# yifangao112/DinoUNet

Hardware: AMD Instinct MI355X
Metric: 2D slices/sec training, dinounet_l 512x512 bf16 (higher is better)
Workload: dtype bf16; 1 GPU; dinounet_l train step (fwd+loss+bwd+clip+SGD), 512x512x3 slices, batch 8/GPU, frozen ViT + adapter + FAPM + U-Net decoder, random-init weights; global_batch=8, parallelism=dp1

## Files before the change

### dinounet_amd/csrc/elementwise.hip

```cpp
#include <stdlib.h>
#include "common.h"
#include "dwconv_plan.h"

namespace {

__host__ int grid_1d(long total) {
  long g = (total + 255) / 256;
  if (g < 1) g = 1;
  if (g > 65535L * 8) g = 65535L * 8;
  return (int)g;
}

#define GRID_STRIDE(i, total) for (long i = (long)blockIdx.x * 256 + threadIdx.x; i < (total); i += (long)gridDim.x * 256)

struct PyrPix { int b, s0, Hs, Ws, yo, xo; };
__device__ __forceinline__ PyrPix pyr_decode(long p, int H, int W) {
  const int n = (H * W) >> 2, N = 21 * n;
  PyrPix q;
  q.b = (int)(p / N);
  int t = (int)(p - (long)q.b * N);
  if (t < 16 * n) { q.s0 = 0; q.Hs = 2 * H; q.Ws = 2 * W; }
  else if (t < 20 * n) { q.s0 = 16 * n; q.Hs = H; q.Ws = W; t -= 16 * n; }
  else { q.s0 = 20 * n; q.Hs = H >> 1; q.Ws = W >> 1; t -= 20 * n; }
  q.yo = t / q.Ws; q.xo = t - q.yo * q.Ws;
// ... 266 lines not shown
  }
}

__global__ __launch_bounds__(256) void dwconv_wgrad_finalize_kernel(const float* __restrict__ part, float* __restrict__ dw,
                                                                    float* __restrict__ db, int blocks, int C, int accum) {
  __shared__ float red[8][33];
  const int col = threadIdx.x & 31, sl = threadIdx.x >> 5;
  const int i = blockIdx.x * 32 + col;
  float acc = 0.f;
  if (i < C * 10)
    for (int b = sl; b < blocks; b += 8) acc += part[(long)b * C * 10 + i];
  red[sl][col] = acc;
  __syncthreads();
  if (sl == 0 && i < C * 10) {
    float t = 0.f;
#pragma unroll
    for (int q = 0; q < 8; q++) t += red[q][col];
    const int k = i / C, c = i - k * C;
    if (k < 9) dw[c * 9 + k] = accum ? dw[c * 9 + k] + t : t;
    else if (db) db[c] = accum ? db[c] + t : t;
  }
}

template <typename T>
__global__ __launch_bounds__(256) void maxpool_fwd_kernel(const T* __restrict__ x, T* __restrict__ y, uint8_t* __restrict__ idx,
                                                          int B, int H, int W, int C, int Ho, int Wo, long total) {
  constexpr int V = Elem<T>::VEC;
  const int cvn = C / V;
  GRID_STRIDE(i, total) {
    const int c0 = (int)(i % cvn) * V;
    long t = i / cvn;
    const int xo = (int)(t % Wo); t /= Wo;
    const int yo = (int)(t % Ho);
    const int b = (int)(t / Ho);
    float best[V]; int bi[V];
#pragma unroll
    for (int j = 0; j < V; j++) { best[j] = -INFINITY; bi[j] = 0; }
#pragma unroll
    for (int dy = 0; dy < 3; dy++) {
      const int yi = yo * 2 - 1 + dy;
      if (yi < 0 || yi >= H) continue;
#pragma unroll
      for (int dx = 0; dx < 3; dx++) {
        const int xi = xo * 2 - 1 + dx;
        if (xi < 0 || xi >= W) continue;
        Vec16<T> v = as_vec<T>(*(const uint4*)(x + (((long)b * H + yi) * W + xi) * C + c0));
// ... 1 lines not shown
        for (int j = 0; j < V; j++) {
          float f = to_f32(v.v[j]);
          if (f > best[j]) { best[j] = f; bi[j] = dy * 3 + dx; }
        }
      }
    }
    const long off = (((long)b * Ho + yo) * Wo + xo) * C + c0;
    Vec16<T> o;
#pragma unroll
    for (int j = 0; j < V; j++) o.v[j] = from_f32<T>(best[j]);
    *(uint4*)(y + off) = as_u4(o);
    if (idx) {
#pragma unroll
      for (int j = 0; j < V; j++) idx[off + j] = (uint8_t)bi[j];
    }
  }
}

template <typename T>
__global__ __launch_bounds__(256) void maxpool_bwd_kernel(const uint8_t* __restrict__ idx, const T* __restrict__ dy,
                                                          T* __restrict__ dx, int B, int H, int W, int C, int Ho, int Wo,
                                                          long total) {
  constexpr int V = Elem<T>::VEC;
  const int cvn = C / V;
  GRID_STRIDE(i, total) {
    const int c0 = (int)(i % cvn) * V;
    long t = i / cvn;
    const int xi = (int)(t % W); t /= W;
    const int yi = (int)(t % H);
    const int b = (int)(t / H);
    float acc[V];
#pragma unroll
    for (int j = 0; j < V; j++) acc[j] = 0.f;
#pragma unroll
    for (int dy_ = 0; dy_ < 3; dy_++) {
      const int ty = yi + 1 - dy_;
      if (ty < 0 || (ty & 1)) continue;
      const int yo = ty >> 1;
      if (yo >= Ho) continue;
#pragma unroll
      for (int dx_ = 0; dx_ < 3; dx_++) {
        const int tx = xi + 1 - dx_;
        if (tx < 0 || (tx & 1)) continue;
        const int xo = tx >> 1;
        if (xo >= Wo) continue;
        const long off = (((long)b * Ho + yo) * Wo + xo) * C + c0;
        Vec16<T> g = as_vec<T>(*(const uint4*)(dy + off));
#pragma unroll
        for (int j = 0; j < V; j++)
          if (idx[off + j] == dy_ * 3 + dx_) acc[j] += to_f32(g.v[j]);
      }
    }
    Vec16<T> o;
#pragma unroll
    for (int j = 0; j < V; j++) o.v[j] = from_f32<T>(acc[j]);
    *(uint4*)(dx + (((long)b * H + yi) * W + xi) * C + c0) = as_u4(o);
  }
}

template <typename TS, typename T, int V>
__global__ __launch_bounds__(256) void bilinear_add_kernel(const TS* __restrict__ src, long lds_, const T* __restrict__ base,
                                                           long ldb, T* __restrict__ out, long ldo, int B, int Hs, int Ws, int Ho,
                                                           int Wo, int C, long total) {
  const int cvn = C / V;
  const float sh = (float)Hs / (float)Ho, sw = (float)Ws / (float)Wo;
  auto load = [&](const TS* p, float* v) {
    if constexpr (sizeof(TS) == 2 && V == 8) {
      const bf16x8 t = __builtin_bit_cast(bf16x8, *(const uint4*)p);
#pragma unroll
      for (int j = 0; j < 8; j++) v[j] = (float)t[j];
    } else if constexpr (sizeof(TS) == 4 && V % 4 == 0) {
#pragma unroll
      for (int j = 0; j < V; j += 4) { const float4 t = *(const float4*)(p + j); v[j] = t.x; v[j + 1] = t.y; v[j + 2] = t.z; v[j + 3] = t.w; }
    } else {
// ... 294 lines not shown
__global__ __launch_bounds__(256) void se_scale_kernel(const T* __restrict__ x, long ldx, const float* __restrict__ gate,
                                                       const T* __restrict__ sc, long ldsc, T* __restrict__ y, long ldy, long P, int C,
                                                       long total) {
  constexpr int V = Elem<T>::VEC;
  const int cvn = C / V;
  GRID_STRIDE(i, total) {
    const int c0 = (int)(i % cvn) * V;
    const long pix = i / cvn;
    const int b = (int)(pix / P);
    Vec16<T> t = as_vec<T>(*(const uint4*)(x + pix * ldx + c0));
    Vec16<T> o;
    if (sc) {
      Vec16<T> s2 = as_vec<T>(*(const uint4*)(sc + pix * ldsc + c0));
#pragma unroll
      for (int j = 0; j < V; j++) o.v[j] = from_f32<T>(to_f32(t.v[j]) * gate[(long)b * C + c0 + j] + to_f32(s2.v[j]));
    } else {
#pragma unroll
      for (int j = 0; j < V; j++) o.v[j] = from_f32<T>(to_f32(t.v[j]) * gate[(long)b * C + c0 + j]);
    }
    *(uint4*)(y + pix * ldy + c0) = as_u4(o);
  }
}

__global__ __launch_bounds__(1024) void se_gate_bwd_kernel(const float* __restrict__ dsum, const float* __restrict__ sums, float invP,
                                                           const float* __restrict__ gate, const float* __restrict__ hidden,
                                                           const float* __restrict__ W1, const float* __restrict__ W2,
                                                           float* __restrict__ dpool, float* __restrict__ dW1, float* __restrict__ db1,
                                                           float* __restrict__ dW2, float* __restrict__ db2, int B, int C, int R, int Bc) {
  extern __shared__ float sm[];
  float* dgp = sm;
  float* pooled = dgp + Bc * C;
  float* h = pooled + Bc * C;
  float* dhp = h + Bc * R;
  const int tid = threadIdx.x;
  for (int b0 = 0; b0 < B; b0 += Bc) {
    const int nb = min(Bc, B - b0);
    for (int i = tid; i < nb * C; i += 1024) {
      const long gi = (long)b0 * C + i;
      const float g = gate[gi];
      dgp[i] = dsum[gi * 2] * g * (1.f - g);
      pooled[i] = sums[gi * 2] * invP;
    }
    for (int i = tid; i < nb * R; i += 1024) h[i] = hidden[(long)b0 * R + i];
    __syncthreads();
    for (int i = tid; i < nb * R; i += 1024) {
      const int bl = i / R, r = i - bl * R;
      float acc = 0.f;
      for (int c = 0; c < C; c++) acc += W2[c * R + r] * dgp[bl * C + c];
      dhp[i] = h[i] > 0.f ? acc : 0.f;
    }
    __syncthreads();
    for (int i = tid; i < C * R; i += 1024) {
      float a2 = 0.f, a1 = 0.f;
      { const int c = i / R, r = i - c * R; for (int bl = 0; bl < nb; bl++) a2 += dgp[bl * C + c] * h[bl * R + r]; }
      { const int r = i / C, c = i - r * C; for (int bl = 0; bl < nb; bl++) a1 += dhp[bl * R + r] * pooled[bl * C + c]; }
      dW2[i] = b0 ? dW2[i] + a2 : a2;
      dW1[i] = b0 ? dW1[i] + a1 : a1;
    }
    for (int c = tid; c < C; c += 1024) {
      float a = 0.f;
      for (int bl = 0; bl < nb; bl++) a += dgp[bl * C + c];
      db2[c] = b0 ? db2[c] + a : a;
    }
    for (int r = tid; r < R; r += 1024) {
      float a = 0.f;
      for (int bl = 0; bl < nb; bl++) a += dhp[bl * R + r];
      db1[r] = b0 ? db1[r] + a : a;
    }
    for (int i = tid; i < nb * C; i += 1024) {
      const int bl = i / C, c = i - bl * C;
      float acc = 0.f;
      for (int r = 0; r < R; r++) acc += W1[r * C + c] * dhp[bl * R + r];
      dpool[(long)b0 * C + i] = acc * invP;
    }
    __syncthreads();
  }
}

template <typename T>
__global__ __launch_bounds__(256) void se_scale_bwd_kernel(const T* __restrict__ dy, long lddy, const float* __restrict__ gate,
                                                           const float* __restrict__ dpool, T* __restrict__ dx, long lddx, long P,
                                                           int C, long total) {
  constexpr int V = Elem<T>::VEC;
  const int cvn = C / V;
  GRID_STRIDE(i, total) {
    const int c0 = (int)(i % cvn) * V;
    const long pix = i / cvn;
    const int b = (int)(pix / P);
    Vec16<T> t = as_vec<T>(*(const uint4*)(dy + pix * lddy + c0));
    Vec16<T> o;
#pragma unroll
    for (int j = 0; j < V; j++) o.v[j] = from_f32<T>(to_f32(t.v[j]) * gate[(long)b * C + c0 + j] + dpool[(long)b * C + c0 + j]);
    *(uint4*)(dx + pix * lddx + c0) = as_u4(o);
  }
}
// ... 56 lines not shown

void du_dwconv_row_wgrad(const DwconvPlan& plan, int dtype, const void* x, const void* dz, float* dw, float* db, int64_t ld, int64_t bs,
                         int B, int H, int W, int C, float* part, hipStream_t st) {
  if (dtype == DU_BF16) dwconv_row_wgrad_launch<bf16_t>(plan, (const bf16_t*)x, (const bf16_t*)dz, dw, db, ld, bs, B, H, W, C, part, st);
  else dwconv_row_wgrad_launch<float>(plan, (const float*)x, (const float*)dz, dw, db, ld, bs, B, H, W, C, part, st);
  hipLaunchKernelGGL(dwconv_wgrad_finalize_kernel, dim3((C * 10 + 31) / 32), dim3(256), 0, st, (const float*)part, dw, db, plan.rows, C, 0);
}

extern "C" int du_maxpool3x3s2_fwd(int dtype, const void* x, void* y, uint8_t* idx, int B, int H, int W, int C, void* stream) {
  hipStream_t st = (hipStream_t)stream;
  const int v = dtype == DU_BF16 ? 8 : 4;
  if (!x || !y || B <= 0 || C % v) return DU_ERR_BAD_ARG;
  const int Ho = (H + 2 - 3) / 2 + 1, Wo = (W + 2 - 3) / 2 + 1;
  long total = (long)B * Ho * Wo * (C / v);
  DISPATCH_T(dtype,
             hipLaunchKernelGGL(maxpool_fwd_kernel<bf16_t>, dim3(grid_1d(total)), dim3(256), 0, st, (const bf16_t*)x, (bf16_t*)y, idx, B, H, W, C, Ho, Wo, total),
             hipLaunchKernelGGL(maxpool_fwd_kernel<float>, dim3(grid_1d(total)), dim3(256), 0, st, (const float*)x, (float*)y, idx, B, H, W, C, Ho, Wo, total));
  return du_check_launch();
}

extern "C" int du_maxpool3x3s2_bwd(int dtype, const uint8_t* idx, const void* dy, void* dx, int B, int H, int W, int C, void* stream) {
  hipStream_t st = (hipStream_t)stream;
  const int v = dtype == DU_BF16 ? 8 : 4;
  if (!idx || !dy || !dx || B <= 0 || C % v) return DU_ERR_BAD_ARG;
  const int Ho = (H + 2 - 3) / 2 + 1, Wo = (W + 2 - 3) / 2 + 1;
  long total = (long)B * H * W * (C / v);
  DISPATCH_T(dtype,
             hipLaunchKernelGGL(maxpool_bwd_kernel<bf16_t>, dim3(grid_1d(total)), dim3(256), 0, st, idx, (const bf16_t*)dy, (bf16_t*)dx, B, H, W, C, Ho, Wo, total),
             hipLaunchKernelGGL(maxpool_bwd_kernel<float>, dim3(grid_1d(total)), dim3(256), 0, st, idx, (const float*)dy, (float*)dx, B, H, W, C, Ho, Wo, total));
  return du_check_launch();
}

extern "C" int du_bilinear_add_fwd(int src_dtype, int dtype, const void* src, int64_t lds_, const void* base, int64_t ldb, void* out,
                                   int64_t ldo, int B, int Hs, int Ws, int Ho, int Wo, int C, void* stream) {
  hipStream_t st = (hipStream_t)stream;
  if (!src || !out || B <= 0 || C % 4) return DU_ERR_BAD_ARG;
  const bool v8 = dtype == DU_BF16 && C % 8 == 0 && lds_ % 8 == 0 && ldo % 8 == 0 && (!base || ldb % 8 == 0) &&
                  ((((uintptr_t)src) | ((uintptr_t)out) | ((uintptr_t)base)) & 15) == 0;
  const int V = v8 ? 8 : 4;
  long total = (long)B * Ho * Wo * (C / V);
  dim3 g(grid_1d(total)), b(256);
#define BL_LAUNCH(TS, T, VV) hipLaunchKernelGGL((bilinear_add_kernel<TS, T, VV>), g, b, 0, st, (const TS*)src, lds_, (const T*)base, ldb, (T*)out, ldo, B, Hs, Ws, Ho, Wo, C, total)
  if (src_dtype == DU_F32 && dtype == DU_F32) BL_LAUNCH(float, float, 4);
  else if (src_dtype == DU_F32 && dtype == DU_BF16) { if (v8) BL_LAUNCH(float, bf16_t, 8); else BL_LAUNCH(float, bf16_t, 4); }
  else if (src_dtype == DU_BF16 && dtype == DU_BF16) { if (v8) BL_LAUNCH(bf16_t, bf16_t, 8); else BL_LAUNCH(bf16_t, bf16_t, 4); }
  else return DU_ERR_BAD_ARG;
#undef BL_LAUNCH
// ... 170 lines not shown
}

extern "C" int du_se_scale_fwd(int dtype, const void* x, int64_t ldx, const float* gate, const void* shortcut, int64_t ldsc, void* y,
                               int64_t ldy, int B, int64_t P, int C, void* stream) {
  hipStream_t st = (hipStream_t)stream;
  const int v = dtype == DU_BF16 ? 8 : 4;
  if (!x || !gate || !y || B <= 0 || P <= 0 || C % v || ldx % v || ldy % v || (shortcut && ldsc % v)) return DU_ERR_BAD_ARG;
  long total = (long)B * P * (C / v);
  DISPATCH_T(dtype,
             hipLaunchKernelGGL(se_scale_kernel<bf16_t>, dim3(grid_1d(total)), dim3(256), 0, st, (const bf16_t*)x, ldx, gate, (const bf16_t*)shortcut, ldsc, (bf16_t*)y, ldy, (long)P, C, total),
             hipLaunchKernelGGL(se_scale_kernel<float>, dim3(grid_1d(total)), dim3(256), 0, st, (const float*)x, ldx, gate, (const float*)shortcut, ldsc, (float*)y, ldy, (long)P, C, total));
  return du_check_launch();
}

extern "C" int du_se_gate_bwd(const float* dsum, const float* sums, float inv_count, const float* gate, const float* hidden,
                              const float* W1, const float* W2, float* dpool, float* dW1, float* db1, float* dW2, float* db2, int B, int C,
                              int R, void* stream) {
  hipStream_t st = (hipStream_t)stream;
  if (!dsum || !sums || !gate || !hidden || !W1 || !W2 || !dpool || !dW1 || !db1 || !dW2 || !db2 || B <= 0 || C <= 0 || R <= 0)
    return DU_ERR_BAD_ARG;
  int Bc = (int)(8000 / (long)(C + R));
  if (Bc < 1) return DU_ERR_UNSUPPORTED;
  if (Bc > B) Bc = B;
  hipLaunchKernelGGL(se_gate_bwd_kernel, dim3(1), dim3(1024), (size_t)2 * Bc * (C + R) * sizeof(float), st, dsum, sums, inv_count, gate, hidden,
                     W1, W2, dpool, dW1, db1, dW2, db2, B, C, R, Bc);
  return du_check_launch();
}

extern "C" int du_se_scale_bwd(int dtype, const void* dy, int64_t lddy, const float* gate, const float* dpool, void* dx, int64_t lddx,
                               int B, int64_t P, int C, void* stream) {
  hipStream_t st = (hipStream_t)stream;
  const int v = dtype == DU_BF16 ? 8 : 4;
  if (!dy || !gate || !dpool || !dx || B <= 0 || P <= 0 || C % v || lddy % v || lddx % v) return DU_ERR_BAD_ARG;
  long total = (long)B * P * (C / v);
  DISPATCH_T(dtype,
             hipLaunchKernelGGL(se_scale_bwd_kernel<bf16_t>, dim3(grid_1d(total)), dim3(256), 0, st, (const bf16_t*)dy, lddy, gate, dpool, (bf16_t*)dx, lddx, (long)P, C, total),
             hipLaunchKernelGGL(se_scale_bwd_kernel<float>, dim3(grid_1d(total)), dim3(256), 0, st, (const float*)dy, lddy, gate, dpool, (float*)dx, lddx, (long)P, C, total));
  return du_check_launch();
}

namespace {
__global__ __launch_bounds__(256) void window_accumulate_kernel(const float* __restrict__ logits, const float* __restrict__ gauss,
                                                                const int* __restrict__ coords, float* __restrict__ pred,
                                                                float* __restrict__ npred, int nb, int K, int ph, int pw, int D, int H,
                                                                int W) {
  const long per = (long)ph * pw, total = (long)nb * per;
  GRID_STRIDE(i, total) {
    const int b = (int)(i / per);
// ... 315 lines not shown
```

### dinounet_amd/csrc/norm.hip

```cpp
#include "common.h"
#include "ln_bwd_row.h"

int g_ln_rows2 = 1;

namespace {

template <typename TI, typename TO, int MAXV>
__global__ __launch_bounds__(256) void layernorm_fwd_kernel(const TI* __restrict__ x, long ldx, const float* __restrict__ w,
                                                            const float* __restrict__ b, TO* __restrict__ y, long ldy,
                                                            float* __restrict__ mean_out, float* __restrict__ rstd_out,
                                                            long rows, int D, float eps) {
  constexpr int VI = Elem<TI>::VEC;
  const int lane = threadIdx.x & 63;
  const long row = (long)blockIdx.x * 4 + (threadIdx.x >> 6);
  if (row >= rows) return;
  const int nvec = D / VI;
  float v[MAXV][VI];
  float s = 0.f;
#pragma unroll
  for (int i = 0; i < MAXV; i++) {
    int vi = lane + i * 64;
    if (vi < nvec) {
      Vec16<TI> t = as_vec<TI>(*(const uint4*)(x + row * ldx + (long)vi * VI));
#pragma unroll
      for (int j = 0; j < VI; j++) { v[i][j] = to_f32(t.v[j]); s += v[i][j]; }
    } else {
#pragma unroll
      for (int j = 0; j < VI; j++) v[i][j] = 0.f;
    }
  }
  const float mean = wave_sum(s) / (float)D;
  float s2 = 0.f;
#pragma unroll
  for (int i = 0; i < MAXV; i++) {
    int vi = lane + i * 64;
    if (vi < nvec) {
#pragma unroll
      for (int j = 0; j < VI; j++) { float d = v[i][j] - mean; s2 += d * d; }
    }
  }
  const float rstd = rsqrtf(wave_sum(s2) / (float)D + eps);
  if (lane == 0) {
    if (mean_out) mean_out[row] = mean;
    if (rstd_out) rstd_out[row] = rstd;
  }
#pragma unroll
  for (int i = 0; i < MAXV; i++) {
    int vi = lane + i * 64;
    if (vi < nvec) {
      const int c0 = vi * VI;
#pragma unroll
      for (int j = 0; j < VI; j++) y[row * ldy + c0 + j] = from_f32<TO>((v[i][j] - mean) * rstd * w[c0 + j] + b[c0 + j]);
    }
  }
}

template <typename TI, typename TO, int MAXV>
__global__ __launch_bounds__(256) void layernorm_fwd2_kernel(const TI* __restrict__ x, long ldx, const float* __restrict__ w,
                                                             const float* __restrict__ b, TO* __restrict__ y, long ldy,
                                                             float* __restrict__ mean_out, float* __restrict__ rstd_out,
                                                             long rows, int D, float eps) {
  constexpr int VI = Elem<TI>::VEC;
  const int lane = threadIdx.x & 63;
  const long row0 = ((long)blockIdx.x * 4 + (threadIdx.x >> 6)) * 2;
  if (row0 >= rows) return;
  const bool two = row0 + 1 < rows;
  const int nvec = D / VI;
  float v[2][MAXV][VI];
  float s[2] = {0.f, 0.f};
#pragma unroll
  for (int u = 0; u < 2; u++)
#pragma unroll
    for (int i = 0; i < MAXV; i++) {
      const int vi = lane + i * 64;
      if (vi < nvec && (u == 0 || two)) {
        Vec16<TI> t = as_vec<TI>(*(const uint4*)(x + (row0 + u) * ldx + (long)vi * VI));
#pragma unroll
        for (int j = 0; j < VI; j++) { v[u][i][j] = to_f32(t.v[j]); s[u] += v[u][i][j]; }
      } else {
#pragma unroll
        for (int j = 0; j < VI; j++) v[u][i][j] = 0.f;
      }
    }
  float mean[2], rstd[2];
#pragma unroll
  for (int u = 0; u < 2; u++) mean[u] = wave_sum(s[u]) / (float)D;
#pragma unroll
  for (int u = 0; u < 2; u++) {
    float s2 = 0.f;
#pragma unroll
    for (int i = 0; i < MAXV; i++) {
      const int vi = lane + i * 64;
      if (vi < nvec) {
#pragma unroll
        for (int j = 0; j < VI; j++) { const float d = v[u][i][j] - mean[u]; s2 += d * d; }
      }
    }
    rstd[u] = rsqrtf(wave_sum(s2) / (float)D + eps);
  }
  if (lane == 0) {
    if (mean_out) { mean_out[row0] = mean[0]; if (two) mean_out[row0 + 1] = mean[1]; }
    if (rstd_out) { rstd_out[row0] = rstd[0]; if (two) rstd_out[row0 + 1] = rstd[1]; }
  }
#pragma unroll
  for (int i = 0; i < MAXV; i++) {
    const int vi = lane + i * 64;
    if (vi < nvec) {
      const int c0 = vi * VI;
#pragma unroll
      for (int u = 0; u < 2; u++) {
        if (u == 1 && !two) break;
#pragma unroll
        for (int j = 0; j < VI; j++) y[(row0 + u) * ldy + c0 + j] = from_f32<TO>((v[u][i][j] - mean[u]) * rstd[u] * w[c0 + j] + b[c0 + j]);
      }
    }
  }
}

template <typename T, int MAXV>
__global__ __launch_bounds__(256) void layernorm_bwd_dx_kernel(const T* __restrict__ x, const T* __restrict__ dy,
                                                               const float* __restrict__ w, const float* __restrict__ mean,
                                                               const float* __restrict__ rstd, T* __restrict__ dx, long rows, int D,
                                                               const T* __restrict__ dres) {
  constexpr int VI = Elem<T>::VEC;
  const int lane = threadIdx.x & 63;
  const long row = (long)blockIdx.x * 4 + (threadIdx.x >> 6);
  if (row >= rows) return;
  const int nvec = D / VI;
  const float mu = mean[row], rs = rstd[row];
  float xh[MAXV][VI], g[MAXV][VI];
  float c1 = 0.f, c2 = 0.f;
#pragma unroll
  for (int i = 0; i < MAXV; i++) {
    int vi = lane + i * 64;
    if (vi < nvec) {
      Vec16<T> tx = as_vec<T>(*(const uint4*)(x + row * (long)D + (long)vi * VI));
// ... 565 lines not shown
  if (i >= n) return;
  const float m = sums[i * 2] * inv_count;
  float var = sums[i * 2 + 1] * inv_count - m * m;
  var = var > 0.f ? var : 0.f;
  mean[i] = m;
  rstd[i] = rsqrtf(var + eps);
  if (run_mean) {
    run_mean[i] = (1.f - momentum) * run_mean[i] + momentum * m;
    run_var[i] = (1.f - momentum) * run_var[i] + momentum * var * unbias;
  }
}

__global__ __launch_bounds__(256) void norm_param_grads_kernel(const float* __restrict__ bs, float* __restrict__ dw, float* __restrict__ db,
                                                               int G, int C) {
  const int c = blockIdx.x * 256 + threadIdx.x;
  if (c >= C) return;
  float a = 0.f, b = 0.f;
  for (int g = 0; g < G; g++) { b += bs[((long)g * C + c) * 2]; a += bs[((long)g * C + c) * 2 + 1]; }
  dw[c] = a; db[c] = b;
}

int grid_for(long total) { long g = (total + 255) / 256; return (int)(g > 8192 ? 8192 : (g < 1 ? 1 : g)); }

template <typename TI, typename TO>
int ln_fwd_dispatch(const void* x, long ldx, const float* w, const float* b, void* y, long ldy, float* m, float* r, long rows,
                    int D, float eps, hipStream_t st) {
  const int nvec = D / Elem<TI>::VEC;
  const int maxv = (nvec + 63) / 64;
  dim3 grid((unsigned)((rows + 3) / 4)), block(256);
  static int wave_slots = 0;
  if (!wave_slots) {
    int dev = 0; hipDeviceProp_t prop;
    wave_slots = (hipGetDevice(&dev) == hipSuccess && hipGetDeviceProperties(&prop, dev) == hipSuccess) ? 32 * prop.multiProcessorCount : 8192;
  }
  if (g_ln_rows2 && maxv <= 4 && (g_ln_rows2 > 1 || (rows > wave_slots && rows <= 2L * wave_slots))) {
    dim3 grid2((unsigned)((rows + 7) / 8));
#define LN2_LAUNCH(MV) hipLaunchKernelGGL((layernorm_fwd2_kernel<TI, TO, MV>), grid2, block, 0, st, (const TI*)x, ldx, w, b, (TO*)y, ldy, m, r, rows, D, eps)
    if (maxv <= 1) LN2_LAUNCH(1); else if (maxv <= 2) LN2_LAUNCH(2); else LN2_LAUNCH(4);
#undef LN2_LAUNCH
    return du_check_launch();
  }
#define LN_LAUNCH(MV) hipLaunchKernelGGL((layernorm_fwd_kernel<TI, TO, MV>), grid, block, 0, st, (const TI*)x, ldx, w, b, (TO*)y, ldy, m, r, rows, D, eps)
  if (maxv <= 1) LN_LAUNCH(1); else if (maxv <= 2) LN_LAUNCH(2); else if (maxv <= 4) LN_LAUNCH(4);
  else if (maxv <= 8) LN_LAUNCH(8); else if (maxv <= 16) LN_LAUNCH(16); else return DU_ERR_UNSUPPORTED;
#undef LN_LAUNCH
  return du_check_launch();
}

template <typename T>
int ln_bwd_dispatch(const void* x, const void* dy, const float* w, const float* mean, const float* rstd, void* dx, float* dwdb,
                    long rows, int D, float* ws, long ws_elems, const void* dres, hipStream_t st) {
  const int nvec = D / Elem<T>::VEC;
  const int maxv = (nvec + 63) / 64;
  dim3 grid((unsigned)((rows + 3) / 4)), block(256);
  {
    static const bool off = DU_GETENV("DU_LN_BWD_FUSED") && atoi(DU_GETENV("DU_LN_BWD_FUSED")) == 0;
    const int STRIP = pick_strip(1, rows, D, Elem<T>::VEC);
    const long strips = (rows + STRIP - 1) / STRIP;
    const size_t lds = (size_t)3 * D * 2 * sizeof(float);
    if (!off && maxv <= 4 && ws && ws_elems >= strips * D * 2 && lds <= 64 * 1024) {
      return strip_launch(dwdb, ws, ws_elems, 1, strips, D, st, [&](float* part) {
#define LNF_LAUNCH(MV) hipLaunchKernelGGL((layernorm_bwd_fused_kernel<T, MV>), dim3((unsigned)strips), block, lds, st, (const T*)x, (const T*)dy, w, mean, rstd, (T*)dx, rows, D, (const T*)dres, STRIP, part)
        if (maxv <= 1) LNF_LAUNCH(1); else if (maxv <= 2) LNF_LAUNCH(2); else LNF_LAUNCH(4);
#undef LNF_LAUNCH
      }, 2);
// ... 11 lines not shown
}

}

int du_norm_finalize_planar(const float* part, float* out, int strips, int C, hipStream_t st) {
  if ((long)C * 2 >= 4096) hipLaunchKernelGGL(finalize_kernel<32>, dim3((unsigned)((C * 2 + 31) / 32)), dim3(256), 0, st, part, out, 1, strips, C * 2, 2);
  else hipLaunchKernelGGL(finalize_kernel<4>, dim3((unsigned)((C * 2 + 3) / 4)), dim3(256), 0, st, part, out, 1, strips, C * 2, 2);
  return du_check_launch();
}

extern "C" int du_layernorm_fwd(int in_dtype, int out_dtype, const void* x, int64_t ldx, const float* w, const float* b, void* y,
                                int64_t ldy, float* mean_out, float* rstd_out, int64_t rows, int D, float eps, void* stream) {
  hipStream_t st = (hipStream_t)stream;
  if (rows <= 0 || D <= 0 || !x || !y || !w || !b) return DU_ERR_BAD_ARG;
  const int vi = in_dtype == DU_BF16 ? 8 : 4;
  if (D % vi || ldx % vi) return DU_ERR_BAD_ARG;
  if (in_dtype == DU_F32 && out_dtype == DU_F32) return ln_fwd_dispatch<float, float>(x, ldx, w, b, y, ldy, mean_out, rstd_out, rows, D, eps, st);
  if (in_dtype == DU_F32 && out_dtype == DU_BF16) return ln_fwd_dispatch<float, bf16_t>(x, ldx, w, b, y, ldy, mean_out, rstd_out, rows, D, eps, st);
  if (in_dtype == DU_BF16 && out_dtype == DU_BF16) return ln_fwd_dispatch<bf16_t, bf16_t>(x, ldx, w, b, y, ldy, mean_out, rstd_out, rows, D, eps, st);
  if (in_dtype == DU_BF16 && out_dtype == DU_F32) return ln_fwd_dispatch<bf16_t, float>(x, ldx, w, b, y, ldy, mean_out, rstd_out, rows, D, eps, st);
  return DU_ERR_BAD_ARG;
}

extern "C" int du_strip_finalize(const float* part, float* out, int G, int strips, int C, void* stream) {
  hipStream_t st = (hipStream_t)stream;
  if (!part || !out || G <= 0 || strips <= 0 || C <= 0) return DU_ERR_BAD_ARG;
  if ((long)G * C * 2 >= 4096) {
    const int chunks = (C * 2 + 31) / 32;
    hipLaunchKernelGGL(finalize_kernel<32>, dim3((unsigned)(G * chunks)), dim3(256), 0, st, part, out, G, strips, C * 2, 0);
  } else {
    const int chunks = (C * 2 + 3) / 4;
    hipLaunchKernelGGL(finalize_kernel<4>, dim3((unsigned)(G * chunks)), dim3(256), 0, st, part, out, G, strips, C * 2, 0);
  }
  return du_check_launch();
}

extern "C" int64_t du_reduce_ws_elems(int dtype, int G, int64_t P, int C) {
  const int v = dtype == DU_BF16 ? 8 : 4;
  if (G <= 0 || P <= 0 || C <= 0 || C % v) return 0;
  const int STRIP = pick_strip(G, P, C, v);
  return (int64_t)G * ((P + STRIP - 1) / STRIP) * C * 2;
}

extern "C" int du_layernorm_bwd(int dtype, const void* x, const void* dy, const float* w, const float* mean, const float* rstd,
                                void* dx, float* dwdb, int64_t rows, int D, float* ws, int64_t ws_elems, const void* dres, void* stream) {
  hipStream_t st = (hipStream_t)stream;
// ... 177 lines not shown
```

### dinounet_amd/dinov3/vision_transformer.py

```python
import math
import os

import numpy as np
import torch
from torch import nn

from .. import ops
from .._lib import ACT_GELU

VIT_CONFIGS = {
    "dinounet_s": dict(embed_dim=384, depth=12, num_heads=6, ffn_layer="mlp", ffn_ratio=4.0, qkv_bias=True),
    "dinounet_b": dict(embed_dim=768, depth=12, num_heads=12, ffn_layer="mlp", ffn_ratio=4.0, qkv_bias=True),
    "dinounet_l": dict(embed_dim=1024, depth=24, num_heads=16, ffn_layer="mlp", ffn_ratio=4.0, qkv_bias=True),
    "dinounet_7b": dict(embed_dim=4096, depth=40, num_heads=32, ffn_layer="swiglu64", ffn_ratio=3.0, qkv_bias=False,
                        untie_global_and_local_cls_norm=True, drop_path_rate=0.4),
}


class LinearKMaskedBias(nn.Linear):

    def __init__(self, *a, **k):
        super().__init__(*a, **k)
        if self.bias is not None:
            self.register_buffer("bias_mask", torch.full_like(self.bias, fill_value=math.nan))
# ... 202 lines not shown
        take = list(n)
        sin_all, cos_all = self.rope_embed.sincos_all(hp, wp, x.device, self.training, len(pk["blocks"]))
        rope_grid = (hp, wp)
        sd = self.training and self.drop_path_rate > 0.0
        k_sub = max(int(B * (1 - self.drop_path_rate)), 1)
        if sd:
            alpha = torch.full((1,), B / k_sub, dtype=torch.float32, device=x.device)

        def attn_branch(xr, Bs, i, d, scale, ws):
            h, _, _ = ops.layernorm_raw(xr, d["n1w"], d["n1b"], 1e-5, dtype)
            a = ops.qkv_attention(h, d["qkv_w"], d["qkv_b"], sin_all[i], cos_all[i], Bs, N, nh, dh, npre, ws, grid=rope_grid)
            ops.mm(a, d["proj_w"], bias=d["proj_b"], gamma=d["g1"], residual=xr, out=xr, row_scale=scale, rs_rows=xr.shape[0] if scale is not None else 0)

        def ffn_branch(xr, d, scale):
            h, _, _ = ops.layernorm_raw(xr, d["n2w"], d["n2b"], 1e-5, dtype)
            rs = xr.shape[0] if scale is not None else 0
            if "fc1_w" in d:
                u = ops.mm(h, d["fc1_w"], bias=d["fc1_b"], act=ACT_GELU)
                ops.mm(u, d["fc2_w"], bias=d["fc2_b"], gamma=d["g2"], residual=xr, out=xr, row_scale=scale, rs_rows=rs)
            else:
                u = ops.mm_swiglu(h, d["w12"], d["b12"])
                ops.mm(u, d["w3"], bias=d["b3"], gamma=d["g2"], residual=xr, out=xr, row_scale=scale, rs_rows=rs)

        taps = [torch.empty((B, N, D), dtype=dtype, device=x.device) for _ in take]

        def run_chain(b0, b1, ws):
            Bs = b1 - b0
            xc = xs[b0:b1].view(Bs * N, D)
            t = 0
            for i, d in enumerate(pk["blocks"]):
                attn_branch(xc, Bs, i, d, None, ws)
                ffn_branch(xc, d, None)
                if i in take:
                    o = taps[t][b0:b1].view(Bs * N, D)
                    if norm:
                        ops.layernorm_raw(xc, pk["norm_w"], pk["norm_b"], 1e-5, dtype, out=o)
                    else:
                        o.copy_(xc)
                    t += 1
            assert t == len(take), f"only {t} / {len(take)} blocks found"

        nch = self.chains if (x.is_cuda and not sd and ops.PROFILE is None and self.chains > 1 and B >= 2 * self.chains
                              and dtype == torch.bfloat16) else 1
        pending = []
        if sd:
            x2 = xs.view(B * N, D)
            t = 0
            for i, d in enumerate(pk["blocks"]):
                if self.pinned_subsets is not None:
                    i1, i2 = (t_.to(x.device) for t_ in self.pinned_subsets[i])
                else:
                    i1 = torch.randperm(B, device=x.device)[:k_sub]
                    i2 = torch.randperm(B, device=x.device)[:k_sub]
                xsub = ops.sample_gather(xs, i1)
                attn_branch(xsub.view(k_sub * N, D), k_sub, i, d, alpha, self._ws)
                ops.sample_scatter_(xs, xsub, i1)
                xsub = ops.sample_gather(xs, i2)
                ffn_branch(xsub.view(k_sub * N, D), d, alpha)
                ops.sample_scatter_(xs, xsub, i2)
                if i in take:
                    o = taps[t].view(B * N, D)
                    if norm:
                        ops.layernorm_raw(x2, pk["norm_w"], pk["norm_b"], 1e-5, dtype, out=o)
                    else:
                        o.copy_(x2)
                    t += 1
            assert t == len(take), f"only {t} / {len(take)} blocks found"
        elif nch == 1:
            run_chain(0, B, self._ws)
        else:
            main = torch.cuda.current_stream()
            key = str(x.device)
            if key not in self._chain_streams:
                self._chain_streams[key] = [torch.cuda.Stream(device=x.device) for _ in range(8)]
            per = (B + nch - 1) // nch
            ops.set_corun(nch)
            try:
                for c in range(nch):
                    b0, b1 = c * per, min(B, (c + 1) * per)
                    if b0 >= b1:
                        continue
                    st = self._chain_streams[key][c]
                    st.wait_stream(main)
                    with torch.cuda.stream(st):
                        run_chain(b0, b1, self._chain_ws.setdefault((key, c), {}))
                    pending.append(st)
            finally:
                ops.set_corun(1)

        keep = [xs, sin_all, cos_all, cols, tok]

        def join():
            if pending:
                cur = torch.cuda.current_stream()
                for st in pending:
                    cur.wait_stream(st)
                pending.clear()
            keep.clear()
            outs = [(o[:, npre:].contiguous(), o[:, 0].contiguous()) for o in taps]
            return tuple(outs) if return_class_token else tuple(o for o, _ in outs)

        return join


def build_backbone(model_name: str) -> DinoVisionTransformer:
    return DinoVisionTransformer(**VIT_CONFIGS[model_name])
```

### dinounet_amd/ops.py

```python
import ctypes as C
import math
import os
import weakref

import torch

from . import _lib
from ._lib import (ACT_GELU, ACT_LEAKY, ACT_NONE, ACT_RELU, ACT_SWIGLU, DU_BF16, DU_F32, IM2COL_COL, IM2COL_ROW, PLAIN_COL,
                   PLAIN_ROW, STORE_MSDA_PREP, STORE_PIXEL_SHUFFLE2, STORE_QKV_HEADS, STORE_QKV_ROPE, STORE_SLABS, ConvGeom, GemmArgs)

__all__ = ["mm", "linear", "conv2d", "conv_transpose2x2", "norm_act", "layer_norm", "msda", "dwconv3x3",
           "maxpool3x3s2", "bilinear_add", "bilinear_resize", "squeeze_excite", "dice_ce_loss", "dice_ce_masked_loss", "dice_bce_loss",
           "labels_to_regions", "val_dice_ce", "val_dice_bce", "ds_seg_loss", "downsample_seg"]


def _code(dt):
    if dt == torch.bfloat16:
        return DU_BF16
    if dt == torch.float32:
        return DU_F32
    raise RuntimeError(f"dinounet_amd: unsupported dtype {dt} (bf16 / fp32 only)")


def _req(*ts):
# ... 1518 lines not shown
        return (None, None, None, *dxs, *dws, *dbs, None)


def sync_bn_multi(xs, bns, act, group):
    n = len(xs)
    mods = [(bn.eps, bn.running_mean, bn.running_var, bn.momentum if bn.momentum is not None else 0.1) for bn in bns]
    return list(_SyncBNMulti.apply(group, act, n, *xs, *[bn.weight for bn in bns], *[bn.bias for bn in bns], mods))


def layernorm_raw(x2d, w, b, eps, out_dtype, want_stats=False, out=None):
    rows, D, ld = _rows2d(x2d)
    if out is None:
        y = torch.empty((rows, D), dtype=out_dtype, device=x2d.device)
    else:
        y = out
        assert y.shape == (rows, D) and y.dtype == out_dtype and y.is_contiguous()
    mean = rstd = None
    if want_stats:
        mean = torch.empty(rows, dtype=torch.float32, device=x2d.device)
        rstd = torch.empty(rows, dtype=torch.float32, device=x2d.device)
    _lib.check(_lib.lib().du_layernorm_fwd(_code(x2d.dtype), _code(out_dtype), _p(x2d), ld, _p(w), _p(b), _p(y), D, _p(mean),
                                           _p(rstd), rows, D, eps, _st()), "du_layernorm_fwd")
    return y, mean, rstd


class _LayerNorm(torch.autograd.Function):

    @staticmethod
    def forward(ctx, x, w, b, eps, with_res):
        xc = x.contiguous()
        wf, bf = _f32(w), _f32(b)
        y, mean, rstd = layernorm_raw(xc.view(-1, xc.shape[-1]), wf, bf, eps, xc.dtype, True)
        ctx.save_for_backward(xc, wf, mean, rstd)
        ctx.with_res = with_res
        ctx.set_materialize_grads(False)
        if with_res:
            return y.view(x.shape), xc.view(x.shape).view_as(xc)
        return y.view(x.shape)

    @staticmethod
    def backward(ctx, dy, dres=None):
        xc, wf, mean, rstd = ctx.saved_tensors
        D = xc.shape[-1]
        if dy is None:
            return dres, None, None, None, None
        dyc = dy.contiguous()
# ... 1009 lines not shown
```

### include/dinounet_hip.h

```cpp
#ifndef DINOUNET_HIP_H
#define DINOUNET_HIP_H

#include <stdint.h>

#ifdef __cplusplus
extern "C" {
#endif

#define DU_OK 0
#define DU_ERR_BAD_ARG (-1)
#define DU_ERR_UNSUPPORTED (-2)
#define DU_ERR_LAUNCH (-3)

#define DU_F32 0
#define DU_BF16 1

#define DU_PLAIN_ROW 0
#define DU_PLAIN_COL 1
#define DU_IM2COL_ROW 2
#define DU_IM2COL_COL 3

#define DU_ACT_NONE 0
#define DU_ACT_GELU 1
#define DU_ACT_RELU 2
// ... 73 lines not shown
                             const void* w, const void* y, int64_t ldy, int want_stats, int64_t* out, int n);
int du_conv3x3_halo_parts(int C1, int Cin, int Cout, int B, int H, int W);
int du_conv3x3_strip(const void* x, int64_t ldx, const void* x2, int64_t ldx2, int C1, int Cin, int Cout, int B, int H, int W,
                     const void* w, const float* bias, void* y, int64_t ldy, float* stats_part, void* stream);
int du_conv3x3_wgrad_halo(const void* x, int64_t ldx, const void* x2, int64_t ldx2, int C1, int Cin, int Cout, int B, int H, int W,
                          const void* dy, int64_t lddy, float* part, float* dw, int with_db, void* stream);
int du_conv3x3_wgrad_plan_describe(const void* x, int64_t ldx, const void* x2, int64_t ldx2, int C1, int Cin, int Cout, int B, int H, int W,
                                   const void* dy, int64_t lddy, int64_t* out, int n);
int du_conv3x3_wgrad_halo_blocks(int C1, int Cin, int Cout, int B, int H, int W);
int du_strip_finalize(const float* part, float* out, int G, int strips, int C, void* stream);

int du_qkv_rope_split(int dtype, const void* qkv, void* q, void* k, void* v, const float* sin_t, const float* cos_t,
                      int B, int N, int Npad, int H, int Dh, int prefix, float qscale, void* stream);
int du_qkv_rope_split_rows(int dtype, const void* qkv_rows, void* q, void* k, void* v, const float* sin_t, const float* cos_t, int B, int N,
                           int Npad, int H, int Dh, int prefix, float qscale, int64_t m_begin, int m_count, void* stream);
int du_qkv_rope_inplace(int dtype, void* q, void* k, const float* sin_t, const float* cos_t, int B, int N, int Npad, int H, int Dh,
                        int prefix, float qscale, int64_t m_limit, void* stream);
int du_attention_fwd(const void* q, const void* k, const void* v, void* out, int B, int H, int N, int Npad, int Dh,
                     void* stream);
int du_softmax_rows_f32(float* x, int64_t rows, int cols, int64_t ld, void* stream);

int du_layernorm_fwd(int in_dtype, int out_dtype, const void* x, int64_t ldx, const float* w, const float* b, void* y,
                     int64_t ldy, float* mean_out, float* rstd_out, int64_t rows, int D, float eps, void* stream);
int64_t du_reduce_ws_elems(int dtype, int G, int64_t pix_per_group, int C);
int du_layernorm_bwd(int dtype, const void* x, const void* dy, const float* w, const float* mean, const float* rstd,
                     void* dx, float* dwdb, int64_t rows, int D, float* ws, int64_t ws_elems, const void* dres, void* stream);
int du_layernorm_bwd_prod_plan(int dtype, const void* x, const void* G, int64_t ldg, const void* Wt, int64_t ldw, int K, const void* dx,
                               const void* dres, int64_t rows, int D, int64_t* out, int n);
int du_layernorm_bwd_prod(int dtype, const void* x, const void* G, int64_t ldg, const void* Wt, int64_t ldw, int K, const float* w,
                          const float* mean, const float* rstd, void* dx, float* dwdb, int64_t rows, int D, float* ws, int64_t ws_elems,
                          const void* dres, void* stream);

int du_chan_stats(int dtype, const void* x, int64_t ldx, float* sums, int G, int64_t pix_per_group, int C, float* ws,
                  int64_t ws_elems, void* stream);
int du_colsum(int dtype, const void* x, int64_t ldx, float* out, int64_t rows, int C, float* ws, int64_t ws_elems, void* stream);
int du_chan_dot(int dtype, const void* a, int64_t lda, const void* b, int64_t ldb, float* sums, int G, int64_t pix_per_group, int C,
                float* ws, int64_t ws_elems, void* stream);
int du_norm_stats_finalize(const float* sums, float count, float eps, float* mean, float* rstd, int G, int C, float* run_mean,
                           float* run_var, float momentum, void* stream);
int du_norm_param_grads(const float* bsums, float* dw, float* db, int G, int C, void* stream);
int du_chan_stats_norm(int dtype, const void* x, int64_t ldx, float* sums, int G, int64_t pix_per_group, int C, float* ws, int64_t ws_elems,
                       float count, float eps, float* mean, float* rstd, float* run_mean, float* run_var, float momentum, void* stream);
int du_strip_finalize_norm(const float* part, float* sums, int G, int strips, int C, float count, float eps, float* mean, float* rstd,
                           float* run_mean, float* run_var, float momentum, void* stream);
int du_norm_act_bwd_stats_grads(int dtype, const void* x, int64_t ldx, const void* dy, int64_t lddy, const float* mean, const float* rstd,
                                const float* w, const float* b, float* bsums, float* dw, float* db, int G, int64_t pix_per_group, int C,
// ... 229 lines not shown
```

Before: 313.6 slices/s.

## Vectorise maxpool backward, stage SE weights in LDS, fuse LN taps split

Three separate changes. The maxpool backward kernel now computes the up-to-4 contributing output windows directly and loads each argmax index as one word, replacing nine branchy taps with byte-wise index loads. The single-block SE gate backward kernel stages W1/W2 in LDS when they fit, and otherwise unrolls its global dot-product loads. The ViT tap layernorm writes patch and class-token rows straight into separate output buffers, removing the later slice-and-contiguous copies. Together these add alignment preconditions and extra code paths.

```diff
diff --git a/dinounet_amd/csrc/elementwise.hip b/dinounet_amd/csrc/elementwise.hip
--- a/dinounet_amd/csrc/elementwise.hip
+++ b/dinounet_amd/csrc/elementwise.hip
@@ -312,6 +312,10 @@
   }
 }
 
+template <int V> struct IdxWord;
+template <> struct IdxWord<8> { using type = unsigned long long; };
+template <> struct IdxWord<4> { using type = unsigned int; };
+
 template <typename T>
 __global__ __launch_bounds__(256) void maxpool_fwd_kernel(const T* __restrict__ x, T* __restrict__ y, uint8_t* __restrict__ idx,
                                                           int B, int H, int W, int C, int Ho, int Wo, long total) {
@@ -359,6 +363,7 @@
                                                           T* __restrict__ dx, int B, int H, int W, int C, int Ho, int Wo,
                                                           long total) {
   constexpr int V = Elem<T>::VEC;
+  using word_t = typename IdxWord<V>::type;
   const int cvn = C / V;
   GRID_STRIDE(i, total) {
     const int c0 = (int)(i % cvn) * V;
@@ -366,27 +371,39 @@
     const int xi = (int)(t % W); t /= W;
     const int yi = (int)(t % H);
     const int b = (int)(t / H);
+    int ky[2], kx[2], wy[2], wx[2];
+    bool vy[2], vx[2];
+#pragma unroll
+    for (int a = 0; a < 2; a++) {
+      ky[a] = (yi & 1) ? 2 * a : 1;
+      wy[a] = (yi + 1 - ky[a]) >> 1;
+      vy[a] = (a == 0 || (yi & 1)) && wy[a] < Ho;
+      kx[a] = (xi & 1) ? 2 * a : 1;
+      wx[a] = (xi + 1 - kx[a]) >> 1;
+      vx[a] = (a == 0 || (xi & 1)) && wx[a] < Wo;
+    }
+    uint4 g[4];
+    word_t w[4];
+#pragma unroll
+    for (int s = 0; s < 4; s++) {
+      g[s] = make_uint4(0u, 0u, 0u, 0u);
+      w[s] = ~(word_t)0;
+      if (vy[s >> 1] && vx[s & 1]) {
+        const long off = (((long)b * Ho + wy[s >> 1]) * Wo + wx[s & 1]) * C + c0;
+        g[s] = *(const uint4*)(dy + off);
+        w[s] = *(const word_t*)(idx + off);
+      }
+    }
     float acc[V];
 #pragma unroll
     for (int j = 0; j < V; j++) acc[j] = 0.f;
 #pragma unroll
-    for (int dy_ = 0; dy_ < 3; dy_++) {
-      const int ty = yi + 1 - dy_;
-      if (ty < 0 || (ty & 1)) continue;
-      const int yo = ty >> 1;
-      if (yo >= Ho) continue;
-#pragma unroll
-      for (int dx_ = 0; dx_ < 3; dx_++) {
-        const int tx = xi + 1 - dx_;
-        if (tx < 0 || (tx & 1)) continue;
-        const int xo = tx >> 1;
-        if (xo >= Wo) continue;
-        const long off = (((long)b * Ho + yo) * Wo + xo) * C + c0;
-        Vec16<T> g = as_vec<T>(*(const uint4*)(dy + off));
-#pragma unroll
-        for (int j = 0; j < V; j++)
-          if (idx[off + j] == dy_ * 3 + dx_) acc[j] += to_f32(g.v[j]);
-      }
+    for (int s = 0; s < 4; s++) {
+      const Vec16<T> gv = as_vec<T>(g[s]);
+      const unsigned k = (unsigned)(ky[s >> 1] * 3 + kx[s & 1]);
+#pragma unroll
+      for (int j = 0; j < V; j++)
+        if ((unsigned)((w[s] >> (8 * j)) & 0xffu) == k) acc[j] += to_f32(gv.v[j]);
     }
     Vec16<T> o;
 #pragma unroll
@@ -727,17 +744,24 @@
   }
 }
 
+constexpr int SE_DOT_U = 64;
+constexpr int SE_STAGE_MAX = 4096;
+template <bool STAGE>
 __global__ __launch_bounds__(1024) void se_gate_bwd_kernel(const float* __restrict__ dsum, const float* __restrict__ sums, float invP,
                                                            const float* __restrict__ gate, const float* __restrict__ hidden,
                                                            const float* __restrict__ W1, const float* __restrict__ W2,
                                                            float* __restrict__ dpool, float* __restrict__ dW1, float* __restrict__ db1,
                                                            float* __restrict__ dW2, float* __restrict__ db2, int B, int C, int R, int Bc) {
   extern __shared__ float sm[];
-  float* dgp = sm;
+  float* W1s = sm;
+  float* W2s = sm + C * R;
+  float* dgp = STAGE ? sm + 2 * C * R : sm;
   float* pooled = dgp + Bc * C;
   float* h = pooled + Bc * C;
   float* dhp = h + Bc * R;
   const int tid = threadIdx.x;
+  float4 w1v = make_float4(0.f, 0.f, 0.f, 0.f), w2v = w1v;
+  if (STAGE && tid * 4 < C * R) { w1v = ((const float4*)W1)[tid]; w2v = ((const float4*)W2)[tid]; }
   for (int b0 = 0; b0 < B; b0 += Bc) {
     const int nb = min(Bc, B - b0);
     for (int i = tid; i < nb * C; i += 1024) {
@@ -747,11 +771,24 @@
       pooled[i] = sums[gi * 2] * invP;
     }
     for (int i = tid; i < nb * R; i += 1024) h[i] = hidden[(long)b0 * R + i];
+    if (STAGE && b0 == 0 && tid * 4 < C * R) { ((float4*)W1s)[tid] = w1v; ((float4*)W2s)[tid] = w2v; }
     __syncthreads();
     for (int i = tid; i < nb * R; i += 1024) {
       const int bl = i / R, r = i - bl * R;
       float acc = 0.f;
-      for (int c = 0; c < C; c++) acc += W2[c * R + r] * dgp[bl * C + c];
+      if constexpr (STAGE) {
+        for (int c = 0; c < C; c++) acc += W2s[c * R + r] * dgp[bl * C + c];
+      } else {
+        int c = 0;
+        for (; c + SE_DOT_U <= C; c += SE_DOT_U) {
+          float wv[SE_DOT_U];
+#pragma unroll
+          for (int j = 0; j < SE_DOT_U; j++) wv[j] = W2[(c + j) * R + r];
+#pragma unroll
+          for (int j = 0; j < SE_DOT_U; j++) acc += wv[j] * dgp[bl * C + c + j];
+        }
+        for (; c < C; c++) acc += W2[c * R + r] * dgp[bl * C + c];
+      }
       dhp[i] = h[i] > 0.f ? acc : 0.f;
     }
     __syncthreads();
@@ -775,7 +812,19 @@
     for (int i = tid; i < nb * C; i += 1024) {
       const int bl = i / C, c = i - bl * C;
       float acc = 0.f;
-      for (int r = 0; r < R; r++) acc += W1[r * C + c] * dhp[bl * R + r];
+      if constexpr (STAGE) {
+        for (int r = 0; r < R; r++) acc += W1s[r * C + c] * dhp[bl * R + r];
+      } else {
+        int r = 0;
+        for (; r + 16 <= R; r += 16) {
+          float wv[16];
+#pragma unroll
+          for (int j = 0; j < 16; j++) wv[j] = W1[(r + j) * C + c];
+#pragma unroll
+          for (int j = 0; j < 16; j++) acc += wv[j] * dhp[bl * R + r + j];
+        }
+        for (; r < R; r++) acc += W1[r * C + c] * dhp[bl * R + r];
+      }
       dpool[(long)b0 * C + i] = acc * invP;
     }
     __syncthreads();
@@ -878,7 +927,7 @@
 extern "C" int du_maxpool3x3s2_bwd(int dtype, const uint8_t* idx, const void* dy, void* dx, int B, int H, int W, int C, void* stream) {
   hipStream_t st = (hipStream_t)stream;
   const int v = dtype == DU_BF16 ? 8 : 4;
-  if (!idx || !dy || !dx || B <= 0 || C % v) return DU_ERR_BAD_ARG;
+  if (!idx || !dy || !dx || B <= 0 || C % v || (uintptr_t)idx % v) return DU_ERR_BAD_ARG;
   const int Ho = (H + 2 - 3) / 2 + 1, Wo = (W + 2 - 3) / 2 + 1;
   long total = (long)B * H * W * (C / v);
   DISPATCH_T(dtype,
@@ -1095,8 +1144,10 @@
   int Bc = (int)(8000 / (long)(C + R));
   if (Bc < 1) return DU_ERR_UNSUPPORTED;
   if (Bc > B) Bc = B;
-  hipLaunchKernelGGL(se_gate_bwd_kernel, dim3(1), dim3(1024), (size_t)2 * Bc * (C + R) * sizeof(float), st, dsum, sums, inv_count, gate, hidden,
-                     W1, W2, dpool, dW1, db1, dW2, db2, B, C, R, Bc);
+  const size_t lds = (size_t)2 * Bc * (C + R) * sizeof(float), wlds = (size_t)2 * C * R * sizeof(float);
+  const bool stage = (long)C * R <= SE_STAGE_MAX && ((long)C * R) % 4 == 0 && lds + wlds <= 64 * 1024 && ((((uintptr_t)W1) | ((uintptr_t)W2)) & 15) == 0;
+  if (stage) hipLaunchKernelGGL(se_gate_bwd_kernel<true>, dim3(1), dim3(1024), lds + wlds, st, dsum, sums, inv_count, gate, hidden, W1, W2, dpool, dW1, db1, dW2, db2, B, C, R, Bc);
+  else hipLaunchKernelGGL(se_gate_bwd_kernel<false>, dim3(1), dim3(1024), lds, st, dsum, sums, inv_count, gate, hidden, W1, W2, dpool, dW1, db1, dW2, db2, B, C, R, Bc);
   return du_check_launch();
 }
 
diff --git a/dinounet_amd/csrc/norm.hip b/dinounet_amd/csrc/norm.hip
--- a/dinounet_amd/csrc/norm.hip
+++ b/dinounet_amd/csrc/norm.hip
@@ -5,15 +5,26 @@
 
 namespace {
 
-template <typename TI, typename TO, int MAXV>
+template <typename TO>
+__device__ __forceinline__ TO* ln_tap_row(TO* y, TO* cls, int D, int s, int t, int N, int npre) {
+  if (t == 0) return cls + (long)s * D;
+  if (t < npre) return nullptr;
+  return y + ((long)s * (N - npre) + (t - npre)) * D;
+}
+
+template <typename TI, typename TO, int MAXV, bool TAPS = false>
 __global__ __launch_bounds__(256) void layernorm_fwd_kernel(const TI* __restrict__ x, long ldx, const float* __restrict__ w,
                                                             const float* __restrict__ b, TO* __restrict__ y, long ldy,
                                                             float* __restrict__ mean_out, float* __restrict__ rstd_out,
-                                                            long rows, int D, float eps) {
+                                                            long rows, int D, float eps, TO* __restrict__ cls = nullptr, int N = 0,
+                                                            int npre = 0) {
   constexpr int VI = Elem<TI>::VEC;
   const int lane = threadIdx.x & 63;
-  const long row = (long)blockIdx.x * 4 + (threadIdx.x >> 6);
-  if (row >= rows) return;
+  const int tok = blockIdx.x * 4 + (threadIdx.x >> 6);
+  const long row = TAPS ? (long)blockIdx.y * N + tok : (long)blockIdx.x * 4 + (threadIdx.x >> 6);
+  if (TAPS ? tok >= N : row >= rows) return;
+  TO* yr = nullptr;
+  if constexpr (TAPS) yr = ln_tap_row(y, cls, D, (int)blockIdx.y, tok, N, npre);
   const int nvec = D / VI;
   float v[MAXV][VI];
   float s = 0.f;
@@ -44,27 +55,40 @@
     if (mean_out) mean_out[row] = mean;
     if (rstd_out) rstd_out[row] = rstd;
   }
+  if (TAPS && !yr) return;
 #pragma unroll
   for (int i = 0; i < MAXV; i++) {
     int vi = lane + i * 64;
     if (vi < nvec) {
       const int c0 = vi * VI;
-#pragma unroll
-      for (int j = 0; j < VI; j++) y[row * ldy + c0 + j] = from_f32<TO>((v[i][j] - mean) * rstd * w[c0 + j] + b[c0 + j]);
-    }
-  }
-}
-
-template <typename TI, typename TO, int MAXV>
+      if constexpr (TAPS) {
+#pragma unroll
+        for (int j = 0; j < VI; j++) yr[c0 + j] = from_f32<TO>((v[i][j] - mean) * rstd * w[c0 + j] + b[c0 + j]);
+      } else {
+#pragma unroll
+        for (int j = 0; j < VI; j++) y[row * ldy + c0 + j] = from_f32<TO>((v[i][j] - mean) * rstd * w[c0 + j] + b[c0 + j]);
+      }
+    }
+  }
+}
+
+template <typename TI, typename TO, int MAXV, bool TAPS = false>
 __global__ __launch_bounds__(256) void layernorm_fwd2_kernel(const TI* __restrict__ x, long ldx, const float* __restrict__ w,
                                                              const float* __restrict__ b, TO* __restrict__ y, long ldy,
                                                              float* __restrict__ mean_out, float* __restrict__ rstd_out,
-                                                             long rows, int D, float eps) {
+                                                             long rows, int D, float eps, TO* __restrict__ cls = nullptr, int N = 0,
+                                                             int npre = 0) {
   constexpr int VI = Elem<TI>::VEC;
   const int lane = threadIdx.x & 63;
-  const long row0 = ((long)blockIdx.x * 4 + (threadIdx.x >> 6)) * 2;
-  if (row0 >= rows) return;
-  const bool two = row0 + 1 < rows;
+  const int tok0 = (blockIdx.x * 4 + (threadIdx.x >> 6)) * 2;
+  const long row0 = TAPS ? (long)blockIdx.y * N + tok0 : ((long)blockIdx.x * 4 + (threadIdx.x >> 6)) * 2;
+  if (TAPS ? tok0 >= N : row0 >= rows) return;
+  const bool two = TAPS ? tok0 + 1 < N : row0 + 1 < rows;
+  TO* yr[2] = {nullptr, nullptr};
+  if constexpr (TAPS) {
+    yr[0] = ln_tap_row(y, cls, D, (int)blockIdx.y, tok0, N, npre);
+    if (two) yr[1] = ln_tap_row(y, cls, D, (int)blockIdx.y, tok0 + 1, N, npre);
+  }
   const int nvec = D / VI;
   float v[2][MAXV][VI];
   float s[2] = {0.f, 0.f};
@@ -109,9 +133,15 @@
       const int c0 = vi * VI;
 #pragma unroll
       for (int u = 0; u < 2; u++) {
-        if (u == 1 && !two) break;
-#pragma unroll
-        for (int j = 0; j < VI; j++) y[(row0 + u) * ldy + c0 + j] = from_f32<TO>((v[u][i][j] - mean[u]) * rstd[u] * w[c0 + j] + b[c0 + j]);
+        if constexpr (TAPS) {
+          if (!yr[u]) continue;
+#pragma unroll
+          for (int j = 0; j < VI; j++) yr[u][c0 + j] = from_f32<TO>((v[u][i][j] - mean[u]) * rstd[u] * w[c0 + j] + b[c0 + j]);
+        } else {
+          if (u == 1 && !two) break;
+#pragma unroll
+          for (int j = 0; j < VI; j++) y[(row0 + u) * ldy + c0 + j] = from_f32<TO>((v[u][i][j] - mean[u]) * rstd[u] * w[c0 + j] + b[c0 + j]);
+        }
       }
     }
   }
@@ -723,12 +753,13 @@
 
 int grid_for(long total) { long g = (total + 255) / 256; return (int)(g > 8192 ? 8192 : (g < 1 ? 1 : g)); }
 
-template <typename TI, typename TO>
+template <typename TI, typename TO, bool TAPS = false>
 int ln_fwd_dispatch(const void* x, long ldx, const float* w, const float* b, void* y, long ldy, float* m, float* r, long rows,
-                    int D, float eps, hipStream_t st) {
+                    int D, float eps, hipStream_t st, void* cls = nullptr, int N = 0, int npre = 0) {
   const int nvec = D / Elem<TI>::VEC;
   const int maxv = (nvec + 63) / 64;
   dim3 grid((unsigned)((rows + 3) / 4)), block(256);
+  if (TAPS) grid = dim3((unsigned)((N + 3) / 4), (unsigned)(rows / N));
   static int wave_slots = 0;
   if (!wave_slots) {
     int dev = 0; hipDeviceProp_t prop;
@@ -736,12 +767,13 @@
   }
   if (g_ln_rows2 && maxv <= 4 && (g_ln_rows2 > 1 || (rows > wave_slots && rows <= 2L * wave_slots))) {
     dim3 grid2((unsigned)((rows + 7) / 8));
-#define LN2_LAUNCH(MV) hipLaunchKernelGGL((layernorm_fwd2_kernel<TI, TO, MV>), grid2, block, 0, st, (const TI*)x, ldx, w, b, (TO*)y, ldy, m, r, rows, D, eps)
+    if (TAPS) grid2 = dim3((unsigned)((N + 7) / 8), (unsigned)(rows / N));
+#define LN2_LAUNCH(MV) hipLaunchKernelGGL((layernorm_fwd2_kernel<TI, TO, MV, TAPS>), grid2, block, 0, st, (const TI*)x, ldx, w, b, (TO*)y, ldy, m, r, rows, D, eps, (TO*)cls, N, npre)
     if (maxv <= 1) LN2_LAUNCH(1); else if (maxv <= 2) LN2_LAUNCH(2); else LN2_LAUNCH(4);
 #undef LN2_LAUNCH
     return du_check_launch();
   }
-#define LN_LAUNCH(MV) hipLaunchKernelGGL((layernorm_fwd_kernel<TI, TO, MV>), grid, block, 0, st, (const TI*)x, ldx, w, b, (TO*)y, ldy, m, r, rows, D, eps)
+#define LN_LAUNCH(MV) hipLaunchKernelGGL((layernorm_fwd_kernel<TI, TO, MV, TAPS>), grid, block, 0, st, (const TI*)x, ldx, w, b, (TO*)y, ldy, m, r, rows, D, eps, (TO*)cls, N, npre)
   if (maxv <= 1) LN_LAUNCH(1); else if (maxv <= 2) LN_LAUNCH(2); else if (maxv <= 4) LN_LAUNCH(4);
   else if (maxv <= 8) LN_LAUNCH(8); else if (maxv <= 16) LN_LAUNCH(16); else return DU_ERR_UNSUPPORTED;
 #undef LN_LAUNCH
@@ -799,6 +831,21 @@
   return DU_ERR_BAD_ARG;
 }
 
+extern "C" int du_layernorm_fwd_taps(int in_dtype, int out_dtype, const void* x, int64_t ldx, const float* w, const float* b, void* patch_out,
+                                     void* cls_out, float* mean_out, float* rstd_out, int64_t rows, int D, int N, int npre, float eps,
+                                     void* stream) {
+  hipStream_t st = (hipStream_t)stream;
+  if (rows <= 0 || D <= 0 || !x || !patch_out || !cls_out || !w || !b) return DU_ERR_BAD_ARG;
+  if (N <= 0 || npre < 1 || npre > N || rows % N || rows / N > 65535) return DU_ERR_BAD_ARG;
+  const int vi = in_dtype == DU_BF16 ? 8 : 4;
+  if (D % vi || ldx % vi) return DU_ERR_BAD_ARG;
+  if (in_dtype == DU_F32 && out_dtype == DU_F32) return ln_fwd_dispatch<float, float, true>(x, ldx, w, b, patch_out, D, mean_out, rstd_out, rows, D, eps, st, cls_out, N, npre);
+  if (in_dtype == DU_F32 && out_dtype == DU_BF16) return ln_fwd_dispatch<float, bf16_t, true>(x, ldx, w, b, patch_out, D, mean_out, rstd_out, rows, D, eps, st, cls_out, N, npre);
+  if (in_dtype == DU_BF16 && out_dtype == DU_BF16) return ln_fwd_dispatch<bf16_t, bf16_t, true>(x, ldx, w, b, patch_out, D, mean_out, rstd_out, rows, D, eps, st, cls_out, N, npre);
+  if (in_dtype == DU_BF16 && out_dtype == DU_F32) return ln_fwd_dispatch<bf16_t, float, true>(x, ldx, w, b, patch_out, D, mean_out, rstd_out, rows, D, eps, st, cls_out, N, npre);
+  return DU_ERR_BAD_ARG;
+}
+
 extern "C" int du_strip_finalize(const float* part, float* out, int G, int strips, int C, void* stream) {
   hipStream_t st = (hipStream_t)stream;
   if (!part || !out || G <= 0 || strips <= 0 || C <= 0) return DU_ERR_BAD_ARG;
diff --git a/dinounet_amd/dinov3/vision_transformer.py b/dinounet_amd/dinov3/vision_transformer.py
--- a/dinounet_amd/dinov3/vision_transformer.py
+++ b/dinounet_amd/dinov3/vision_transformer.py
@@ -248,7 +248,10 @@
                 u = ops.mm_swiglu(h, d["w12"], d["b12"])
                 ops.mm(u, d["w3"], bias=d["b3"], gamma=d["g2"], residual=xr, out=xr, row_scale=scale, rs_rows=rs)
 
-        taps = [torch.empty((B, N, D), dtype=dtype, device=x.device) for _ in take]
+        if norm:
+            taps = [(torch.empty((B, hp * wp, D), dtype=dtype, device=x.device), torch.empty((B, D), dtype=dtype, device=x.device)) for _ in take]
+        else:
+            taps = [torch.empty((B, N, D), dtype=dtype, device=x.device) for _ in take]
 
         def run_chain(b0, b1, ws):
             Bs = b1 - b0
@@ -258,11 +261,10 @@
                 attn_branch(xc, Bs, i, d, None, ws)
                 ffn_branch(xc, d, None)
                 if i in take:
-                    o = taps[t][b0:b1].view(Bs * N, D)
                     if norm:
-                        ops.layernorm_raw(xc, pk["norm_w"], pk["norm_b"], 1e-5, dtype, out=o)
+                        ops.layernorm_taps(xc, pk["norm_w"], pk["norm_b"], 1e-5, N, npre, taps[t][0][b0:b1], taps[t][1][b0:b1])
                     else:
-                        o.copy_(xc)
+                        taps[t][b0:b1].view(Bs * N, D).copy_(xc)
                     t += 1
             assert t == len(take), f"only {t} / {len(take)} blocks found"
 
@@ -285,11 +287,10 @@
                 ffn_branch(xsub.view(k_sub * N, D), d, alpha)
                 ops.sample_scatter_(xs, xsub, i2)
                 if i in take:
-                    o = taps[t].view(B * N, D)
                     if norm:
-                        ops.layernorm_raw(x2, pk["norm_w"], pk["norm_b"], 1e-5, dtype, out=o)
+                        ops.layernorm_taps(x2, pk["norm_w"], pk["norm_b"], 1e-5, N, npre, *taps[t])
                     else:
-                        o.copy_(x2)
+                        taps[t].view(B * N, D).copy_(x2)
                     t += 1
             assert t == len(take), f"only {t} / {len(take)} blocks found"
         elif nch == 1:
@@ -323,7 +324,7 @@
                     cur.wait_stream(st)
                 pending.clear()
             keep.clear()
-            outs = [(o[:, npre:].contiguous(), o[:, 0].contiguous()) for o in taps]
+            outs = list(taps) if norm else [(o[:, npre:].contiguous(), o[:, 0].contiguous()) for o in taps]
             return tuple(outs) if return_class_token else tuple(o for o, _ in outs)
 
         return join
diff --git a/dinounet_amd/ops.py b/dinounet_amd/ops.py
--- a/dinounet_amd/ops.py
+++ b/dinounet_amd/ops.py
@@ -1564,6 +1564,20 @@
     _lib.check(_lib.lib().du_layernorm_fwd(_code(x2d.dtype), _code(out_dtype), _p(x2d), ld, _p(w), _p(b), _p(y), D, _p(mean),
                                            _p(rstd), rows, D, eps, _st()), "du_layernorm_fwd")
     return y, mean, rstd
+
+
+def layernorm_taps(x2d, w, b, eps, N, npre, patch_out, cls_out):
+    rows, D, ld = _rows2d(x2d)
+    Bs = rows // N
+    assert rows == Bs * N and patch_out.shape == (Bs, N - npre, D) and cls_out.shape == (Bs, D)
+    assert patch_out.dtype == cls_out.dtype and patch_out.is_contiguous() and cls_out.is_contiguous()
+    if not x2d.is_cuda:
+        o = layernorm_raw(x2d, w, b, eps, patch_out.dtype)[0].view(Bs, N, D)
+        patch_out.copy_(o[:, npre:])
+        cls_out.copy_(o[:, 0])
+        return
+    _lib.check(_lib.lib().du_layernorm_fwd_taps(_code(x2d.dtype), _code(patch_out.dtype), _p(x2d), ld, _p(w), _p(b), _p(patch_out), _p(cls_out),
+                                                None, None, rows, D, N, npre, eps, _st()), "du_layernorm_fwd_taps")
 
 
 class _LayerNorm(torch.autograd.Function):
diff --git a/include/dinounet_hip.h b/include/dinounet_hip.h
--- a/include/dinounet_hip.h
+++ b/include/dinounet_hip.h
@@ -119,6 +119,8 @@
 
 int du_layernorm_fwd(int in_dtype, int out_dtype, const void* x, int64_t ldx, const float* w, const float* b, void* y,
                      int64_t ldy, float* mean_out, float* rstd_out, int64_t rows, int D, float eps, void* stream);
+int du_layernorm_fwd_taps(int in_dtype, int out_dtype, const void* x, int64_t ldx, const float* w, const float* b, void* patch_out,
+                          void* cls_out, float* mean_out, float* rstd_out, int64_t rows, int D, int N, int npre, float eps, void* stream);
 int64_t du_reduce_ws_elems(int dtype, int G, int64_t pix_per_group, int C);
 int du_layernorm_bwd(int dtype, const void* x, const void* dy, const float* w, const float* mean, const float* rstd,
                      void* dx, float* dwdb, int64_t rows, int D, float* ws, int64_t ws_elems, const void* dres, void* stream);
```

Result: no change. 315.8 slices/s, median of 6 (+0.7%).
